# ROAM-Lab-ND/generalized_rbda

Hardware: AMD Instinct MI355X
Metric: forward-dynamics evals/sec (batched random states), MIT Humanoid cluster model (higher is better)
Workload: dtype f32; 1 GPU; mit_humanoid.urdf cluster-ABA, 262144 random states per GPU; batch_per_gpu=262144, batch_global=262144, nq=25, nv=24, n_bodies=37, n_clusters=17, parallelism=batch-sharded x1, plan replicated

## Files before the change

generalized_rbda_amd/csrc/capi.cpp:

```cpp
#include <hip/hip_runtime.h>

#include <array>
#include <cassert>
#include <cmath>
#include <cstdio>
#include <cstdlib>
#include <cstring>
#include <map>
#include <memory>
#include <mutex>
#include <string>
#include <vector>

#include "../../include/grbda_hip.h"
#include "../../include/grbda_hip_vjp.h"
#include "../../include/grbda_hip_step_vjp.h"
#include "../../include/grbda_hip_jvp.h"
#include "../../include/grbda_hip_wrench.h"
#include "../../include/grbda_hip_bodies.h"
#include "../../include/grbda_hip_jacobians.h"
#include "../../include/grbda_hip_jacobian_products.h"
#include "../../include/grbda_model_desc.h"
#include "devplan.h"

// ... 605 lines not shown
        if (int rc = ensure_scratch(p, device, stream, scratch_bytes(grid, static_cast<size_t>(d.n_glb_slots) + in_rows, sizeof(T)), &scratch)) return rc;
        hipError_t e = launch_aba_chain_lm<T>(d, q, qd, tau, ydd, B, static_cast<T *>(scratch), static_cast<int>(grid), lds_lm, hs, r.lm_waves);
        return e == hipSuccess ? GRBDA_OK : hip_err(e, "aba chain launch (latency mode)");
    }
    const int kid = sizeof(T) == 8 ? 1 : 0;
    const size_t waves_per_cu = static_cast<size_t>((sizeof(T) == 8 && !cp.gens.empty()) ? p->opt.waves_per_cu_f64_wide_regs : p->opt.waves_per_cu[kid]);
    const LaunchShape s = launch_shape(t.n_cu, n_tiles, waves_per_cu, static_cast<size_t>(cp.n_lds) * kWave * sizeof(T), h.nq, h.nv, sizeof(T),
                                       static_cast<size_t>(p->opt.lds_bytes_per_wave[kid]), true);
    {
        int n_free_bwd = 0, at_bwd = -1;
        for (size_t i = 0; i < cp.segs.size(); i++)
            if (cp.segs[i].op == SEG_FREE_BWD) { n_free_bwd++; at_bwd = static_cast<int>(i); }
        if (!cp.segs.empty() && cp.segs[0].op == SEG_FREE_FWD && n_free_bwd == 1 && cp.frees[cp.segs[0].first].lds_v >= 0) {
            if (s.stage_all_fits) d.fuse |= 1;
            d.stage_lds_v = cp.frees[cp.segs[0].first].lds_v;
            d.stage_v_index = cp.frees[cp.segs[0].first].v_index;
        }
        if (n_free_bwd == 1 && at_bwd + 1 < static_cast<int>(cp.segs.size()) && cp.segs[at_bwd + 1].op == SEG_FREE_ACC &&
            cp.segs[at_bwd + 1].first == cp.segs[at_bwd].first)
            d.fuse |= 2;
    }
    d.lds_bytes = static_cast<int>(s.lds_bytes);
    const bool inreg = !wrenches && chain_inputs_in_registers(sizeof(T), d.n_gens, d.n_diffs, d.sv_global, d.nq, d.nv);
    if (inreg) d.direct_in = chain_direct_inputs(sizeof(T), d.nq, d.nv, q, qd, tau);
    const size_t slab_rows = static_cast<size_t>(chain_slab_rows(inreg, d.nq, d.nv, d.n_glb_slots, d.out_lds).total);
    if (int rc = ensure_scratch(p, device, stream, scratch_bytes(s.grid, slab_rows, sizeof(T)), &scratch)) return rc;
    hipError_t e = wrenches ? launch_aba_chain_wrench<T>(d, *wrenches, q, qd, tau, ydd, B, static_cast<T *>(scratch), static_cast<int>(s.grid), s.lds_bytes, hs)
                            : launch_aba_chain<T>(d, q, qd, tau, ydd, B, static_cast<T *>(scratch), static_cast<int>(s.grid), s.lds_bytes, hs);
    return e == hipSuccess ? GRBDA_OK : hip_err(e, "aba chain launch");
}

template <class T>
int run_rnea_chain(const grbda_plan *p, const DeviceTables &t, const Route &r, const T *q, const T *qd, const T *ydd, T *tau, size_t B, int device,
                   void *stream, bool gravity = true, const WrenchList<T> *wrenches = nullptr)
{
    const HostPlan &h = p->host;
    const RneaChainProgram &rp = h.rchain[r.slot];
    const size_t n_tiles = (B + kWave - 1) / kWave;
    const size_t in_rows = static_cast<size_t>(h.nq + 2 * h.nv);
    const hipStream_t hs = static_cast<hipStream_t>(stream);
    RneaChainDev<T> d = rnea_chain_dev<T>(p, t, r.slot);
    if (!gravity)
        for (int i = 0; i < 6; i++) d.a_root[i] = T(0);
    void *scratch = nullptr;
    if (r.path == ROUTE_LM) {
        if (rp.diffs.empty()) d.diffs = nullptr;
        no_gens(d);
// ... 4045 lines not shown
```

generalized_rbda_amd/csrc/chain_kernels.hip:

```cpp
#include <hip/hip_runtime.h>

#include "devplan.h"

#ifndef GRBDA_CHAIN_UNIT
#define GRBDA_CHAIN_UNIT 0
#endif
#define GRBDA_KLDS (GRBDA_CHAIN_UNIT == 3)

namespace grbda_hip {

#include "devmath.h"

template <class T>
struct ChainTables {
    cptr<ChainSeg> segs;
    cptr<ChainLink> links;
    cptr<ChainPair> pairs;
    cptr<ChainFree> frees;
    cptr<ChainDiff> diffs;
    cptr<ChainGen> gens;
    cptr<ChainGenBody> gbodies;
    cptr<int32_t> cints;
    cptr<T> consts;
    int n_segs, nq, nv, ori_repr;
// ... 88 lines not shown
        if constexpr (sizeof(T) == 4) {
            if (out_row >= 0) reinterpret_cast<T *>(grbda_smem)[(out_row + j) * kWave + lane] = v;
            else put(j, v);
        } else {
            out_f[j * kWave + lane] = v;
        }
    }
    T *out_f;
    __device__ __forceinline__ void set_out(int row)
    {
        out_row = row;
        out_f = row >= 0 ? reinterpret_cast<T *>(grbda_smem) + row * kWave : out_u;
    }
    __device__ __forceinline__ void put(int j, T v) const
    {
        *reinterpret_cast<T *>(reinterpret_cast<char *>(out_u + (size_t)(unsigned)(j * kWave)) + (size_t)lane_b) = v;
    }
    __device__ __forceinline__ void wrench(int, T (&)[6]) const {}
};

template <class T>
struct ChainMemR : ChainMem<T> {
    typedef T Row __attribute__((ext_vector_type(kInRegCols)));
    Row rq, rqd, rx;
    __device__ __forceinline__ T q(int j) const { return rq[j]; }
    __device__ __forceinline__ T qd(int j) const { return rqd[j]; }
    __device__ __forceinline__ T x(int j) const { return rx[j]; }
};

template <class T>
struct ChainMemW : ChainMem<T> {
    int wbody[kMaxWrenches];
    unsigned wcanon;
    const T *wl;
    __device__ __forceinline__ void wrench(int body, T (&p)[6]) const
    {
        unsigned hits = 0;
#pragma unroll
        for (int i = 0; i < kMaxWrenches; i++) hits |= (wbody[i] == body ? 1u : 0u) << i;
        while (hits) {
            const int i = __builtin_ctz(hits);
            hits &= hits - 1;
            const T *w = wl + i * 6;
            const int shift = (int)((wcanon >> (2 * i)) & 3u) + 1;
#pragma unroll
            for (int j = 0; j < 3; j++) {
                const int k = (j + shift) % 3;
                p[j] -= w[k];
                p[3 + j] -= w[3 + k];
            }
// ... 343 lines not shown
#pragma unroll
    for (int j = 0; j < 6; j++) solve2(F0[j], F1[j], blk[j], blk[6 + j]);
    solve2(u[0], u[1], blk[12], blk[13]);
    M.glb_st(pr.glb_k, blk);
    if constexpr (OSIM) {
        const T ex[7] = {i00, i01, i11, s1, c1, s2, c2};
        M.glb_st(pr.glb_k + 14, ex);
    }
#pragma unroll
    for (int r = 0; r < 6; r++) {
        psi[r] += F0[r] * blk[12] + F1[r] * blk[13];
#pragma unroll
        for (int cc = r; cc < 6; cc++) IA[sidx(r, cc)] -= F0[r] * blk[cc] + F1[r] * blk[6 + cc];
    }
}
template <class T, bool OSIM, class MM>
__device__ __forceinline__ void pair_bwd(const ChainTables<T> &P, const MM &M, const ChainPair &pr, T (&IA)[21],
                                         T (&psi)[6])
{
    if (perm_if<T>(kPermPair, pr.perm[0]) == 0 && pr.perm[1] == 0) pair_bwd_k<T, OSIM, 0, 0>(P, M, pr, IA, psi);
    else pair_bwd_k<T, OSIM, -1, -1>(P, M, pr, IA, psi);
}

template <class T>
__device__ __forceinline__ void pair_acc(const ChainTables<T> &P, const ChainMem<T> &M, const ChainPair &pr)
{
    T blk[14], va[12];
    M.glb_ld(pr.glb_k, blk);
    M.lds_ld(pr.lds_pva, va);
    T y0 = blk[12], y1 = blk[13];
#pragma unroll
    for (int j = 0; j < 6; j++) {
        y0 -= blk[j] * va[6 + j];
        y1 -= blk[6 + j] * va[6 + j];
    }
    M.put_f(pr.v_index, y0);
    M.put_f(pr.v_index + 1, y1);
}


template <class T, class TB>
__device__ __forceinline__ void diff_constraint(const TB &P, const ChainMem<T> &M, int tofs_i, int lds_w, const T (&qs)[4], T yd0,
                                                T yd1, T (&X)[4], T (&g)[2], T (&qdl)[2])
{
    cptr<int32_t> ip = P.cints + tofs_i;
    const int n_args = ip[0], n_atoms = ip[1];
    cptr<T> dp = P.consts + ip[2];
    for (int i = 0; i < n_args; i++) {
// ... 542 lines not shown
#pragma unroll
                for (int j = 0; j < 8; j++) blk[j] = blkn[j];
            }
        }
    }
    if (sg.lds_acc_out != -1) {
        T acc[27];
        if (sg.acc_first) {
#pragma unroll
            for (int j = 0; j < 21; j++) acc[j] = IAc[j];
#pragma unroll
            for (int j = 0; j < 6; j++) acc[21 + j] = psic[j];
        } else {
            M.acc_ld(sg.lds_acc_out, acc);
#pragma unroll
            for (int j = 0; j < 21; j++) acc[j] += IAc[j];
#pragma unroll
            for (int j = 0; j < 6; j++) acc[21 + j] += psic[j];
        }
        M.acc_st(sg.lds_acc_out, acc);
    }
}

template <class T>
__device__ __forceinline__ void run_acc(const ChainTables<T> &P, const ChainMem<T> &M, const ChainSeg &sg)
{
    T vp[6], ap[6];
    if (sg.lds_pva >= 0) {
        T va[12];
        M.lds_ld(sg.lds_pva, va);
#pragma unroll
        for (int j = 0; j < 6; j++) {
            vp[j] = va[j];
            ap[j] = va[6 + j];
        }
    } else {
#pragma unroll
        for (int j = 0; j < 6; j++) {
            vp[j] = 0;
            ap[j] = P.a_root[j];
        }
    }
    ChainLink l = load_rec(P.links + sg.first);
    T kb[7];
    M.glb_ld(l.glb_k, kb);
    T yd = M.qd(l.v_index), yq = l.has_child ? M.q(l.q_index) : T(0);
    for (int i = 0; i < sg.count; i++) {
        const bool more = i + 1 < sg.count;
// ... 123 lines not shown
#pragma unroll
                    for (int j = 0; j < 6; j++) {
                        vp[j] = v[j];
                        ap[j] = a[j];
                    }
                }
            }
        }
    }
}

template <class T, class MM>
__device__ __forceinline__ void free_fwd(const ChainTables<T> &P, const MM &M, const ChainFree &f)
{
    if (f.lds_v < 0) return;
    T v[6];
#pragma unroll
    for (int j = 0; j < 6; j++) v[j] = M.qd(f.v_index + j);
    M.lds_st(f.lds_v, v);
}

template <class T, class MM>
__device__ __forceinline__ void free_acc_inputs(const ChainTables<T> &P, const MM &M, const ChainFree &f, T (&o)[4], T (&r)[3]);
template <class T>
__device__ __forceinline__ void free_acc_core(const ChainTables<T> &P, const ChainMem<T> &M, const ChainFree &f, const T (&y0)[6],
                                              const T (&o)[4], const T (&r)[3], const T (&vb)[6]);
template <class T, bool OSIM, class MM>
__device__ __forceinline__ void free_bwd(const ChainTables<T> &P, const MM &M, const ChainFree &f, bool fuse_acc = false)
{
    cptr<T> Ic = P.consts + f.bofs;
    cptr<T> Ib = P.consts + f.iofs;
    T v[6], psi[6], IA[21];
#pragma unroll
    for (int j = 0; j < 6; j++) v[j] = M.qd(f.v_index + j);
    T o_[4] = {0, 0, 0, 0}, r_[3] = {0, 0, 0};
    if constexpr (!OSIM) {
        if (fuse_acc) free_acc_inputs(P, M, f, o_, r_);
    }
    bias_force(Ic, v, psi);
    M.wrench(f.body, psi);
    if (f.lds_acc != -1) {
        T acc[27];
        M.acc_ld(f.lds_acc, acc);
#pragma unroll
        for (int j = 0; j < 21; j++) IA[j] = Ib[j] + acc[j];
#pragma unroll
        for (int j = 0; j < 6; j++) psi[j] += acc[21 + j];
        if (f.lds_acc2 != -1) {
// ... 34 lines not shown
    }
    M.glb_st(f.glb_y0, u);
    if constexpr (OSIM) {
        T ex[27];
#pragma unroll
        for (int i = 0; i < 6; i++) {
#pragma unroll
            for (int j = 0; j <= i; j++) ex[i * (i + 1) / 2 + j] = ch.L[i][j];
            ex[21 + i] = ch.inv[i];
        }
        M.glb_st(f.glb_y0 + 6, ex);
    }
}

template <class T, class MM>
__device__ __forceinline__ void free_acc_inputs(const ChainTables<T> &P, const MM &M, const ChainFree &f, T (&o)[4], T (&r)[3])
{
    const int nori = P.ori_repr == 0 ? 4 : 3;
#pragma unroll
    for (int j = 0; j < 4; j++) o[j] = j < nori ? M.q(f.q_index + 3 + j) : T(0);
#pragma unroll
    for (int j = 0; j < 3; j++) r[j] = M.q(f.q_index + j);
}
template <class T>
__device__ __forceinline__ void free_acc_core(const ChainTables<T> &P, const ChainMem<T> &M, const ChainFree &f, const T (&y0)[6],
                                              const T (&o)[4], const T (&r)[3], const T (&vb)[6])
{
    T E[9], g[6], ag[6];
    free_rotation(P.ori_repr, o, E);
#pragma unroll
    for (int j = 0; j < 6; j++) g[j] = P.a_root[j];
    xmotion(E, r, g, ag);
#pragma unroll
    for (int j = 0; j < 6; j++) M.put_f(f.v_index + j, y0[j] - ag[j]);
    if (f.lds_va >= 0) {
        T va[12];
#pragma unroll
        for (int j = 0; j < 6; j++) {
            va[j] = vb[j];
            va[6 + j] = y0[j];
        }
        M.lds_st(f.lds_va, va);
    }
}
template <class T, class MM>
__device__ __forceinline__ void free_acc(const ChainTables<T> &P, const MM &M, const ChainFree &f)
{
    T y0[6], o[4], r[3], vb[6];
// ... 119 lines not shown
template int gen1_waves_per_simd<float>(int);
template int gen1_waves_per_simd<double>(int);
template <class T>
hipError_t launch_aba_gen1(const ChainDev<T> &P, int n, int implicit, const T *q, const T *qd, const T *tau, T *ydd, size_t B, int grid,
                           size_t lds_bytes, hipStream_t stream)
{
    if (implicit) {
        if (n == 1) return launch_gen1<T, 1, true>(P, q, qd, tau, ydd, B, grid, lds_bytes, stream);
        if (n == 2) return launch_gen1<T, 2, true>(P, q, qd, tau, ydd, B, grid, lds_bytes, stream);
        if (n == 3) return launch_gen1<T, 3, true>(P, q, qd, tau, ydd, B, grid, lds_bytes, stream);
        return launch_gen1<T, 4, true>(P, q, qd, tau, ydd, B, grid, lds_bytes, stream);
    }
    if (n == 1) return launch_gen1<T, 1, false>(P, q, qd, tau, ydd, B, grid, lds_bytes, stream);
    if (n == 2) return launch_gen1<T, 2, false>(P, q, qd, tau, ydd, B, grid, lds_bytes, stream);
    if (n == 3) return launch_gen1<T, 3, false>(P, q, qd, tau, ydd, B, grid, lds_bytes, stream);
    return launch_gen1<T, 4, false>(P, q, qd, tau, ydd, B, grid, lds_bytes, stream);
}
template hipError_t launch_aba_gen1<float>(const ChainDev<float> &, int, int, const float *, const float *, const float *, float *, size_t, int,
                                           size_t, hipStream_t);
template hipError_t launch_aba_gen1<double>(const ChainDev<double> &, int, int, const double *, const double *, const double *, double *,
                                            size_t, int, size_t, hipStream_t);
#endif

template <class T, int WPS, int MODE, int DIRECT = 0>
__global__ __launch_bounds__(kWave, WPS) void aba_chain_kernel(ChainDev<T> DP, const T *__restrict__ q, const T *__restrict__ qd,
                                                             const T *__restrict__ tau, T *__restrict__ ydd, size_t B,
                                                             T *__restrict__ scratch)
{
    constexpr bool DIFF = MODE == 1 || MODE == 2, GEN = MODE == 2, INREG = MODE == kModeInReg;
    static_assert(INREG || DIRECT == 0, "direct row loads fill the register vectors of kModeInReg");
    ChainTables<T> P;
    P.segs = (cptr<ChainSeg>)DP.segs;
    P.links = (cptr<ChainLink>)DP.links;
    P.pairs = (cptr<ChainPair>)DP.pairs;
    P.frees = (cptr<ChainFree>)DP.frees;
    P.diffs = DIFF ? (cptr<ChainDiff>)DP.diffs : nullptr;
    P.gens = GEN ? (cptr<ChainGen>)DP.gens : nullptr;
    P.gbodies = GEN ? (cptr<ChainGenBody>)DP.gbodies : nullptr;
    P.cints = DIFF ? (cptr<int32_t>)DP.cints : nullptr;
    P.consts = (cptr<T>)DP.consts;
    P.n_segs = DP.n_segs;
    P.nq = DP.nq;
    P.nv = DP.nv;
    P.ori_repr = DP.ori_repr;
#pragma unroll
    for (int i = 0; i < 6; i++) P.a_root[i] = DP.a_root[i];
    const int lane = threadIdx.x;
    const ChainSlabRows rows = chain_slab_rows(INREG, P.nq, P.nv, DP.n_glb_slots, DP.out_lds);
    T *slab = scratch + (size_t)blockIdx.x * (size_t)rows.total * kWave;
    std::conditional_t<INREG, ChainMemR<T>, ChainMem<T>> M;
    M.lane = lane;
    M.lane_b = (unsigned)lane * (unsigned)sizeof(T);
    M.gmul = 1;
    M.amask = ~0;
    M.glb_u = slab + (size_t)rows.glb * kWave;
    M.in_q_u = slab;
    M.in_qd_u = slab + (size_t)P.nq * kWave;
    M.in_x_u = slab + (size_t)(P.nq + P.nv) * kWave;
    M.out_u = slab + (size_t)rows.out * kWave;
    M.set_out(DP.out_lds);
    M.bad = 0;

    const size_t n_tiles = (B + kWave - 1) / kWave;
    for (size_t tile = blockIdx.x; tile < n_tiles; tile += gridDim.x) {
        const size_t left = B - tile * kWave;
        const int rows_valid = left < (size_t)kWave ? (int)left : kWave;
        if constexpr (INREG)
            stage_inputs_reg<kInRegCols, (DIRECT & kDirectQ) != 0, (DIRECT & kDirectQd) != 0, (DIRECT & kDirectX) != 0>(
                q, qd, tau, tile, rows_valid, P.nq, P.nv, M.rq, M.rqd, M.rx, lane, DP.lds_bytes);
        else stage_inputs(q, qd, tau, tile, rows_valid, P.nq, P.nv, slab, lane, DP.lds_bytes);
        if (DP.fuse & 1) {
            T v[6];
            if constexpr ((DIRECT & kDirectQd) != 0) {
#pragma unroll
                for (int j = 0; j < 6; j++) v[j] = M.rqd[DP.stage_v_index + j];
            } else {
                const T *mine = reinterpret_cast<const T *>(grbda_smem) + (kWave * P.nq + lane * P.nv + DP.stage_v_index);
#pragma unroll
                for (int j = 0; j < 6; j++) v[j] = mine[j];
                wave_lds_fence();
            }
            M.lds_st(DP.stage_lds_v, v);
        }
        for (int s = 0; s < P.n_segs; s++) {
            const ChainSeg sg = load_rec(P.segs + s);
            switch (sg.op) {
                case SEG_RUN_FWD:
                    if (DP.sv_global) run_fwd<T, true>(P, M, sg);
                    else run_fwd_c(P, M, sg);
                    break;
                case SEG_RUN_BWD: {
                    if (DP.sv_global) run_bwd<T, false, true>(P, M, sg);
                    else if (sg.rot_kind == 1) run_bwd<T, false, false, 1>(P, M, sg);
                    else run_bwd<T, false, false>(P, M, sg);
                    break;
                }
// ... 8 lines not shown
                case SEG_DIFF_FWD:
                    if constexpr (DIFF) diff_fwd(P, M, load_rec(P.diffs + sg.first));
                    break;
                case SEG_DIFF_BWD:
                    if constexpr (DIFF) diff_bwd<T, false>(P, M, load_rec(P.diffs + sg.first));
                    break;
                case SEG_DIFF_ACC:
                    if constexpr (DIFF) diff_acc(P, M, load_rec(P.diffs + sg.first));
                    break;
                case SEG_GEN_FWD:
                    if constexpr (GEN) gen_segment<T, 0>(P, M, load_rec(P.gens + sg.first));
                    break;
                case SEG_GEN_BWD:
                    if constexpr (GEN) gen_segment<T, 1>(P, M, load_rec(P.gens + sg.first));
                    break;
                case SEG_GEN_ACC:
                    if constexpr (GEN) gen_segment<T, 2>(P, M, load_rec(P.gens + sg.first));
                    break;
                default:
                    if (!(DP.fuse & 2)) free_acc(P, M, load_rec(P.frees + sg.first));
                    break;
            }
        }
        if (M.out_row >= 0) write_outputs_lds<T>(M.out_row, ydd, tile, rows_valid, P.nv, lane);
        else write_outputs(slab + (size_t)rows.out * kWave, ydd, tile, rows_valid, P.nv, lane);
        M.flush_bad(DP.bad_count, rows_valid);
    }
}


template <class T, int NW, bool DIFF = false>
__global__ __launch_bounds__(NW * kWave) __attribute__((amdgpu_waves_per_eu(2, 2)))
void aba_chain_lm_kernel(ChainDev<T> DP, const T *__restrict__ q, const T *__restrict__ qd, const T *__restrict__ tau,
                         T *__restrict__ ydd, size_t B, T *__restrict__ scratch)
{
    ChainTables<T> P;
    P.segs = (cptr<ChainSeg>)DP.segs;
    P.links = (cptr<ChainLink>)DP.links;
    P.pairs = (cptr<ChainPair>)DP.pairs;
    P.frees = (cptr<ChainFree>)DP.frees;
    P.diffs = DIFF ? (cptr<ChainDiff>)DP.diffs : nullptr;
    P.gens = nullptr;
    P.gbodies = nullptr;
    P.cints = DIFF ? (cptr<int32_t>)DP.cints : nullptr;
    P.consts = (cptr<T>)DP.consts;
    P.n_segs = DP.n_segs;
    P.nq = DP.nq;
// ... 525 lines not shown
                                              double *, double *, size_t, double *, int, size_t, hipStream_t);
#endif

hipError_t launch_aba_chain_diff_f64(const ChainDev<double> &P, const double *q, const double *qd, const double *tau, double *ydd, size_t B,
                                     double *scratch, int grid, size_t lds_bytes, hipStream_t stream);
template <class T>
hipError_t launch_aba_chain_gen(const ChainDev<T> &P, const T *q, const T *qd, const T *tau, T *ydd, size_t B, T *scratch, int grid,
                                size_t lds_bytes, hipStream_t stream);
template <class T>
hipError_t launch_aba_chain(const ChainDev<T> &P, const T *q, const T *qd, const T *tau, T *ydd, size_t B, T *scratch, int grid,
                            size_t lds_bytes, hipStream_t stream)
{
    if (P.n_gens > 0) return launch_aba_chain_gen<T>(P, q, qd, tau, ydd, B, scratch, grid, lds_bytes, stream);
    if (P.n_diffs > 0) {
        if constexpr (sizeof(T) == 8) {
            return launch_aba_chain_diff_f64(P, q, qd, tau, ydd, B, scratch, grid, lds_bytes, stream);
        } else {
            hipLaunchKernelGGL((aba_chain_kernel<T, 2, 1>), dim3(grid), dim3(kWave), lds_bytes, stream, P, q, qd, tau, ydd, B, scratch);
            return hipGetLastError();
        }
    }
    if constexpr (sizeof(T) == 4) {
        if (chain_inputs_in_registers(sizeof(T), P.n_gens, P.n_diffs, P.sv_global, P.nq, P.nv)) {
            if (P.direct_in == (kDirectQ | kDirectQd | kDirectX))
                hipLaunchKernelGGL((aba_chain_kernel<T, 2, kModeInReg, kDirectQ | kDirectQd | kDirectX>), dim3(grid), dim3(kWave), lds_bytes, stream, P, q, qd,
                                   tau, ydd, B, scratch);
            else if (P.direct_in == (kDirectQd | kDirectX))
                hipLaunchKernelGGL((aba_chain_kernel<T, 2, kModeInReg, kDirectQd | kDirectX>), dim3(grid), dim3(kWave), lds_bytes, stream, P, q, qd, tau,
                                   ydd, B, scratch);
            else
                hipLaunchKernelGGL((aba_chain_kernel<T, 2, kModeInReg>), dim3(grid), dim3(kWave), lds_bytes, stream, P, q, qd, tau, ydd, B, scratch);
            return hipGetLastError();
        }
    }
    hipLaunchKernelGGL((aba_chain_kernel<T, 2, 0>), dim3(grid), dim3(kWave), lds_bytes, stream, P, q, qd, tau, ydd, B, scratch);
    return hipGetLastError();
}
#if GRBDA_CHAIN_UNIT == 0
template hipError_t launch_aba_chain<float>(const ChainDev<float> &, const float *, const float *, const float *, float *, size_t,
                                            float *, int, size_t, hipStream_t);
template hipError_t launch_aba_chain<double>(const ChainDev<double> &, const double *, const double *, const double *, double *,
                                             size_t, double *, int, size_t, hipStream_t);
#elif GRBDA_CHAIN_UNIT == 1
hipError_t launch_aba_chain_diff_f64(const ChainDev<double> &P, const double *q, const double *qd, const double *tau, double *ydd, size_t B,
                                     double *scratch, int grid, size_t lds_bytes, hipStream_t stream)
{
    hipLaunchKernelGGL((aba_chain_kernel<double, 2, 1>), dim3(grid), dim3(kWave), lds_bytes, stream, P, q, qd, tau, ydd, B, scratch);
    return hipGetLastError();
}
#elif GRBDA_CHAIN_UNIT == 2
template <class T>
hipError_t launch_aba_chain_gen(const ChainDev<T> &P, const T *q, const T *qd, const T *tau, T *ydd, size_t B, T *scratch, int grid,
                                size_t lds_bytes, hipStream_t stream)
{
// ... 874 lines not shown
                                                    const float *, float *, size_t, float *, int, size_t, hipStream_t);
template hipError_t launch_rnea_chain_wrench<double>(const RneaChainDev<double> &, const WrenchList<double> &, int, const double *, const double *,
                                                     const double *, double *, size_t, double *, int, size_t, hipStream_t);
#endif


static hipError_t set_max_dynamic_lds(const void *const *kernels, int n)
{
    for (int i = 0; i < n; i++) {
        const hipError_t e = hipFuncSetAttribute(kernels[i], hipFuncAttributeMaxDynamicSharedMemorySize, 160 * 1024);
        if (e != hipSuccess) return e;
    }
    return hipSuccess;
}
hipError_t set_max_dynamic_lds_chain_unit1();
hipError_t set_max_dynamic_lds_chain_unit2();
hipError_t set_max_dynamic_lds_chain_unit3();
#if GRBDA_CHAIN_UNIT == 0
hipError_t set_max_dynamic_lds_chain()
{
    const void *const kernels[] = {
        reinterpret_cast<const void *>(&aba_chain_kernel<float, 2, 0>), reinterpret_cast<const void *>(&aba_chain_kernel<float, 2, 1>),
        reinterpret_cast<const void *>(&aba_chain_kernel<float, 2, kModeInReg>),
        reinterpret_cast<const void *>(&aba_chain_kernel<float, 2, kModeInReg, kDirectQd | kDirectX>),
        reinterpret_cast<const void *>(&aba_chain_kernel<float, 2, kModeInReg, kDirectQ | kDirectQd | kDirectX>),
        reinterpret_cast<const void *>(&aba_chain_kernel<double, 2, 0>),
        reinterpret_cast<const void *>(&rnea_chain_kernel<float, 0, false>), reinterpret_cast<const void *>(&rnea_chain_kernel<float, 1, false>),
        reinterpret_cast<const void *>(&rnea_chain_kernel<double, 0, false>), reinterpret_cast<const void *>(&rnea_chain_kernel<double, 1, false>),
        reinterpret_cast<const void *>(&rnea_chain_kernel<float, 0, true>), reinterpret_cast<const void *>(&rnea_chain_kernel<float, 1, true>),
        reinterpret_cast<const void *>(&rnea_chain_kernel<double, 0, true>), reinterpret_cast<const void *>(&rnea_chain_kernel<double, 1, true>),
        reinterpret_cast<const void *>(&osim_chain_kernel<float>), reinterpret_cast<const void *>(&osim_chain_kernel<double>)};
    const hipError_t e = set_max_dynamic_lds(kernels, static_cast<int>(sizeof(kernels) / sizeof(kernels[0])));
    if (e != hipSuccess) return e;
    const hipError_t e1 = set_max_dynamic_lds_chain_unit1();
    if (e1 != hipSuccess) return e1;
    const hipError_t e2 = set_max_dynamic_lds_chain_unit2();
    return e2 != hipSuccess ? e2 : set_max_dynamic_lds_chain_unit3();
}
#elif GRBDA_CHAIN_UNIT == 1
hipError_t set_max_dynamic_lds_chain_unit1()
{
    const void *const kernels[] = {reinterpret_cast<const void *>(&aba_chain_kernel<double, 2, 1>),
                                   reinterpret_cast<const void *>(&aba_chain_lm_kernel<double, 2>)};
    return set_max_dynamic_lds(kernels, 2);
}
#elif GRBDA_CHAIN_UNIT == 3
hipError_t set_max_dynamic_lds_chain_unit3()
{
// ... 31 lines not shown
```

generalized_rbda_amd/csrc/devmath.h:

```cpp
#pragma once

template <class U>
using cptr = const U __attribute__((address_space(4))) *;

template <class U>
__device__ __forceinline__ U load_rec(cptr<U> p)
{
    static_assert(sizeof(U) % 4 == 0, "plan records are arrays of int32");
    U out;
    cptr<int32_t> src = (cptr<int32_t>)p;
    int32_t *dst = reinterpret_cast<int32_t *>(&out);
#pragma unroll
    for (int i = 0; i < (int)(sizeof(U) / 4); i++) dst[i] = src[i];
    return out;
}

extern __shared__ __attribute__((aligned(16))) unsigned char grbda_smem[];

__host__ __device__ constexpr int sidx(int i, int j)
{
    return i <= j ? (i * 6 - i * (i - 1) / 2 + (j - i)) : (j * 6 - j * (j - 1) / 2 + (i - j));
}

template <class T>
// ... 356 lines not shown
        stage_transpose(nq, 0u, slab, lane);
        stage_transpose(nv, bq, slab + (size_t)nq * kWave, lane);
        stage_transpose(nv, bq + bv, slab + (size_t)(nq + nv) * kWave, lane);
        wave_lds_fence();
    } else {
        stage_issue(q, tile, rows_valid, nq, 0u, lane);
        asm volatile("s_waitcnt vmcnt(0)" ::: "memory");
        wave_lds_fence();
        stage_transpose(nq, 0u, slab, lane);
        wave_lds_fence();
        stage_issue(qd, tile, rows_valid, nv, 0u, lane);
        asm volatile("s_waitcnt vmcnt(0)" ::: "memory");
        wave_lds_fence();
        stage_transpose(nv, 0u, slab + (size_t)nq * kWave, lane);
        wave_lds_fence();
        stage_issue(x, tile, rows_valid, nv, 0u, lane);
        asm volatile("s_waitcnt vmcnt(0)" ::: "memory");
        wave_lds_fence();
        stage_transpose(nv, 0u, slab + (size_t)(nq + nv) * kWave, lane);
        wave_lds_fence();
    }
}

template <class T, int N, class ROW>
__device__ __forceinline__ void stage_row_regs(int ncols, unsigned lds_byte_off, ROW &r, int lane)
{
    const T *stage = reinterpret_cast<const T *>(grbda_smem + lds_byte_off);
    constexpr int V = 16 / (int)sizeof(T);
    static_assert(N % V == 0, "whole 16-byte reads");
    if ((ncols % V) == 0 && (lds_byte_off % 16u) == 0) {
        struct alignas(16) Vec { T v[V]; };
        const Vec *rows = reinterpret_cast<const Vec *>(stage + lane * ncols);
#pragma unroll
        for (int c = 0; c < N; c += V) {
            if (c < ncols) {
                const Vec x = rows[c / V];
#pragma unroll
                for (int k = 0; k < V; k++) r[c + k] = x.v[k];
            }
        }
        return;
    }
#pragma unroll
    for (int c = 0; c < N; c++)
        if (c < ncols) r[c] = stage[lane * ncols + c];
}
template <class T, int N, class ROW>
__device__ __forceinline__ void load_row_regs(const T *__restrict__ src, size_t tile, int rows_valid, int ncols, ROW &r, int lane)
{
    constexpr int V = 16 / (int)sizeof(T);
    static_assert(N % V == 0, "whole 16-byte loads");
    struct alignas(16) Vec { T v[V]; };
    const int row = lane < rows_valid ? lane : rows_valid - 1;
    const Vec *mine = reinterpret_cast<const Vec *>(src + (tile * (size_t)kWave + (size_t)row) * (size_t)ncols);
    const int last = ncols / V - 1;
#pragma unroll
    for (int c = 0; c < N; c += V) {
        const Vec x = mine[c / V < last ? c / V : last];
#pragma unroll
        for (int k = 0; k < V; k++) r[c + k] = x.v[k];
    }
}
template <int K>
__device__ __forceinline__ void wait_all_but_youngest()
{
    static_assert(K >= 0 && K < 64, "six bits of vmcnt");
    asm volatile("s_waitcnt vmcnt(%0)" ::"n"(K) : "memory");
}
template <int N, bool DQ, bool DQD, bool DX, class T, class ROW>
__device__ __forceinline__ void stage_inputs_reg(const T *__restrict__ q, const T *__restrict__ qd, const T *__restrict__ x, size_t tile,
                                                 int rows_valid, int nq, int nv, ROW &rq, ROW &rqd, ROW &rx, int lane, int lds_bytes)
{
    constexpr int V = 16 / (int)sizeof(T), kDirectLoads = ((DQ ? 1 : 0) + (DQD ? 1 : 0) + (DX ? 1 : 0)) * (N / V);
    const unsigned bq = (unsigned)(kWave * nq) * (unsigned)sizeof(T), bv = (unsigned)(kWave * nv) * (unsigned)sizeof(T);
    if ((int)(bq + 2 * bv) <= lds_bytes) {
        if constexpr (!DQ) stage_issue(q, tile, rows_valid, nq, 0u, lane);
        if constexpr (!DQD) stage_issue(qd, tile, rows_valid, nv, bq, lane);
        if constexpr (!DX) stage_issue(x, tile, rows_valid, nv, bq + bv, lane);
        if constexpr (kDirectLoads > 0) asm volatile("" ::: "memory");
        if constexpr (DQ) load_row_regs<T, N>(q, tile, rows_valid, nq, rq, lane);
        if constexpr (DQD) load_row_regs<T, N>(qd, tile, rows_valid, nv, rqd, lane);
        if constexpr (DQD && DX) asm volatile("" ::: "memory");
        if constexpr (DX) load_row_regs<T, N>(x, tile, rows_valid, nv, rx, lane);
        if constexpr (DQ && DQD && DX) return;
        wait_all_but_youngest<kDirectLoads>();
        wave_lds_fence();
        if constexpr (!DQ) stage_row_regs<T, N>(nq, 0u, rq, lane);
        if constexpr (!DQD) stage_row_regs<T, N>(nv, bq, rqd, lane);
        if constexpr (!DX) stage_row_regs<T, N>(nv, bq + bv, rx, lane);
        wave_lds_fence();
    } else {
        if constexpr (DQ) load_row_regs<T, N>(q, tile, rows_valid, nq, rq, lane);
        if constexpr (DQD) load_row_regs<T, N>(qd, tile, rows_valid, nv, rqd, lane);
        if constexpr (DX) load_row_regs<T, N>(x, tile, rows_valid, nv, rx, lane);
        if constexpr (!DQ) {
            stage_issue(q, tile, rows_valid, nq, 0u, lane);
            asm volatile("s_waitcnt vmcnt(0)" ::: "memory");
            wave_lds_fence();
            stage_row_regs<T, N>(nq, 0u, rq, lane);
            wave_lds_fence();
        }
        if constexpr (!DQD) {
            stage_issue(qd, tile, rows_valid, nv, 0u, lane);
            asm volatile("s_waitcnt vmcnt(0)" ::: "memory");
            wave_lds_fence();
            stage_row_regs<T, N>(nv, 0u, rqd, lane);
            wave_lds_fence();
        }
        if constexpr (!DX) {
            stage_issue(x, tile, rows_valid, nv, 0u, lane);
            asm volatile("s_waitcnt vmcnt(0)" ::: "memory");
            wave_lds_fence();
            stage_row_regs<T, N>(nv, 0u, rx, lane);
            wave_lds_fence();
        }
    }
}

template <class T>
__device__ __forceinline__ void write_outputs(const T *rows, T *__restrict__ out, size_t tile, int rows_valid, int nv,
                                              int lane)
{
    asm volatile("s_waitcnt vmcnt(0) lgkmcnt(0)" ::: "memory");
    T *stage = reinterpret_cast<T *>(grbda_smem);
    constexpr int V = 16 / (int)sizeof(T);
    if ((nv % V) == 0) {
        struct alignas(16) Vec { T v[V]; };
        Vec *mine = reinterpret_cast<Vec *>(stage + lane * nv);
        for (int c = 0; c < nv; c += V) {
            Vec x;
#pragma unroll
            for (int k = 0; k < V; k++) x.v[k] = rows[(size_t)(c + k) * kWave + lane];
            mine[c / V] = x;
        }
    } else {
        for (int c = 0; c < nv; c++) stage[lane * nv + c] = rows[(size_t)c * kWave + lane];
    }
    wave_lds_fence();
    T *dst = out + tile * (size_t)kWave * (size_t)nv;
// ... 193 lines not shown
```

generalized_rbda_amd/csrc/devplan.h:

```cpp
#pragma once
#include <cstdlib>
#include <hip/hip_runtime.h>

#include "plan.h"
#include "walk.h"

namespace grbda_hip {

inline size_t lds_workgroups_per_cu(size_t lds_bytes)
{
    if (lds_bytes == 0) return 32;
    constexpr size_t granule = 1280;
    return (160u * 1024u) / ((lds_bytes + granule - 1) / granule * granule);
}


template <class T>
struct DevPlan {
    const Step *steps;
    int n_steps;
    const ClusterRec *clusters;
    const BodyRec *bodies;
    const T *consts;
    const int32_t *cints;
// ... 40 lines not shown
template <class T>
hipError_t launch_twists(const DevPlan<T> &P, int n_clusters, int n_span, const T *q, const T *qd_span, const T *qdd_span, T *V, size_t B,
                         int grid, hipStream_t stream);
hipError_t set_max_dynamic_lds();

template <class T>
struct ChainDev {
    const ChainSeg *segs;
    const ChainLink *links;
    const ChainPair *pairs;
    const ChainFree *frees;
    const ChainDiff *diffs;
    int n_diffs;
    const ChainGen *gens;
    const ChainGenBody *gbodies;
    int n_gens;
    const int32_t *cints;
    const T *consts;
    int n_segs;
    int nq, nv;
    int n_glb_slots;
    int lds_bytes;
    int ori_repr;
    int direct_in;
    int sv_global;
    int out_lds;
    int fuse, stage_lds_v, stage_v_index;
    unsigned long long *bad_count;
    T a_root[6];
};
constexpr int kInRegCols = 32;
constexpr int kModeInReg = 3;
inline bool chain_inputs_in_registers(size_t elem, int n_gens, int n_diffs, int sv_global, int nq, int nv)
{
    return elem == 4 && n_gens == 0 && n_diffs == 0 && !sv_global && nq <= kInRegCols && nv <= kInRegCols;
}
constexpr int kDirectQ = 1, kDirectQd = 2, kDirectX = 4;
inline int chain_direct_inputs(size_t elem, int nq, int nv, const void *q, const void *qd, const void *x)
{
    const auto direct = [elem](int ncols, const void *base) {
        return (static_cast<size_t>(ncols) * elem) % 16 == 0 && reinterpret_cast<uintptr_t>(base) % 16 == 0;
    };
    if (!direct(nv, qd) || !direct(nv, x)) return 0;
    return kDirectQd | kDirectX | (direct(nq, q) ? kDirectQ : 0);
}
struct ChainSlabRows {
    int glb;
    int out;
    int total;
};
__host__ __device__ inline ChainSlabRows chain_slab_rows(bool in_registers, int nq, int nv, int n_glb_slots, int out_lds)
{
    if (!in_registers) return {nq + 2 * nv, nq + nv, nq + 2 * nv + n_glb_slots};
    return {0, out_lds < 0 ? n_glb_slots : 0, n_glb_slots + (out_lds < 0 ? nv : 0)};
}
template <class T>
hipError_t launch_aba_chain(const ChainDev<T> &P, const T *q, const T *qd, const T *tau, T *ydd, size_t B, T *scratch, int grid,
                            size_t lds_bytes, hipStream_t stream);
template <class T>
hipError_t launch_aba_chain_lm(const ChainDev<T> &P, const T *q, const T *qd, const T *tau, T *ydd, size_t B, T *scratch, int grid,
                               size_t lds_bytes, hipStream_t stream, int n_waves);
hipError_t set_max_dynamic_lds_chain();
template <class T>
hipError_t launch_aba_gen1(const ChainDev<T> &P, int n, int implicit, const T *q, const T *qd, const T *tau, T *ydd, size_t B, int grid,
                           size_t lds_bytes, hipStream_t stream);
template <class T>
int gen1_waves_per_simd(int n);
// ... 275 lines not shown
```

Baseline: 2.322 billion evals/s.

## Load chain inputs directly into registers and write outputs from registers

Result: faster. 2.481 billion evals/s, median of 6 (+6.9%).

```diff
diff --git a/generalized_rbda_amd/csrc/capi.cpp b/generalized_rbda_amd/csrc/capi.cpp
--- a/generalized_rbda_amd/csrc/capi.cpp
+++ b/generalized_rbda_amd/csrc/capi.cpp
@@ -651,7 +651,6 @@
     }
     d.lds_bytes = static_cast<int>(s.lds_bytes);
     const bool inreg = !wrenches && chain_inputs_in_registers(sizeof(T), d.n_gens, d.n_diffs, d.sv_global, d.nq, d.nv);
-    if (inreg) d.direct_in = chain_direct_inputs(sizeof(T), d.nq, d.nv, q, qd, tau);
     const size_t slab_rows = static_cast<size_t>(chain_slab_rows(inreg, d.nq, d.nv, d.n_glb_slots, d.out_lds).total);
     if (int rc = ensure_scratch(p, device, stream, scratch_bytes(s.grid, slab_rows, sizeof(T)), &scratch)) return rc;
     hipError_t e = wrenches ? launch_aba_chain_wrench<T>(d, *wrenches, q, qd, tau, ydd, B, static_cast<T *>(scratch), static_cast<int>(s.grid), s.lds_bytes, hs)
diff --git a/generalized_rbda_amd/csrc/chain_kernels.hip b/generalized_rbda_amd/csrc/chain_kernels.hip
--- a/generalized_rbda_amd/csrc/chain_kernels.hip
+++ b/generalized_rbda_amd/csrc/chain_kernels.hip
@@ -134,10 +134,14 @@
 template <class T>
 struct ChainMemR : ChainMem<T> {
     typedef T Row __attribute__((ext_vector_type(kInRegCols)));
-    Row rq, rqd, rx;
+    Row rq, rqd;
+    mutable Row rx;
     __device__ __forceinline__ T q(int j) const { return rq[j]; }
     __device__ __forceinline__ T qd(int j) const { return rqd[j]; }
     __device__ __forceinline__ T x(int j) const { return rx[j]; }
+    __device__ __forceinline__ void put_f(int j, T v) const { rx[j] = v; }
+    void put(int, T) const = delete;
+    T got(int) const = delete;
 };
 
 template <class T>
@@ -527,8 +531,8 @@
     else pair_bwd_k<T, OSIM, -1, -1>(P, M, pr, IA, psi);
 }
 
-template <class T>
-__device__ __forceinline__ void pair_acc(const ChainTables<T> &P, const ChainMem<T> &M, const ChainPair &pr)
+template <class T, class MM>
+__device__ __forceinline__ void pair_acc(const ChainTables<T> &P, const MM &M, const ChainPair &pr)
 {
     T blk[14], va[12];
     M.glb_ld(pr.glb_k, blk);
@@ -1117,8 +1121,8 @@
     }
 }
 
-template <class T>
-__device__ __forceinline__ void run_acc(const ChainTables<T> &P, const ChainMem<T> &M, const ChainSeg &sg)
+template <class T, class MM>
+__device__ __forceinline__ void run_acc(const ChainTables<T> &P, const MM &M, const ChainSeg &sg)
 {
     T vp[6], ap[6];
     if (sg.lds_pva >= 0) {
@@ -1288,8 +1292,8 @@
 
 template <class T, class MM>
 __device__ __forceinline__ void free_acc_inputs(const ChainTables<T> &P, const MM &M, const ChainFree &f, T (&o)[4], T (&r)[3]);
-template <class T>
-__device__ __forceinline__ void free_acc_core(const ChainTables<T> &P, const ChainMem<T> &M, const ChainFree &f, const T (&y0)[6],
+template <class T, class MM>
+__device__ __forceinline__ void free_acc_core(const ChainTables<T> &P, const MM &M, const ChainFree &f, const T (&y0)[6],
                                               const T (&o)[4], const T (&r)[3], const T (&vb)[6]);
 template <class T, bool OSIM, class MM>
 __device__ __forceinline__ void free_bwd(const ChainTables<T> &P, const MM &M, const ChainFree &f, bool fuse_acc = false)
@@ -1370,8 +1374,8 @@
 #pragma unroll
     for (int j = 0; j < 3; j++) r[j] = M.q(f.q_index + j);
 }
-template <class T>
-__device__ __forceinline__ void free_acc_core(const ChainTables<T> &P, const ChainMem<T> &M, const ChainFree &f, const T (&y0)[6],
+template <class T, class MM>
+__device__ __forceinline__ void free_acc_core(const ChainTables<T> &P, const MM &M, const ChainFree &f, const T (&y0)[6],
                                               const T (&o)[4], const T (&r)[3], const T (&vb)[6])
 {
     T E[9], g[6], ag[6];
@@ -1537,13 +1541,12 @@
                                             size_t, int, size_t, hipStream_t);
 #endif
 
-template <class T, int WPS, int MODE, int DIRECT = 0>
+template <class T, int WPS, int MODE>
 __global__ __launch_bounds__(kWave, WPS) void aba_chain_kernel(ChainDev<T> DP, const T *__restrict__ q, const T *__restrict__ qd,
                                                              const T *__restrict__ tau, T *__restrict__ ydd, size_t B,
                                                              T *__restrict__ scratch)
 {
     constexpr bool DIFF = MODE == 1 || MODE == 2, GEN = MODE == 2, INREG = MODE == kModeInReg;
-    static_assert(INREG || DIRECT == 0, "direct row loads fill the register vectors of kModeInReg");
     ChainTables<T> P;
     P.segs = (cptr<ChainSeg>)DP.segs;
     P.links = (cptr<ChainLink>)DP.links;
@@ -1580,13 +1583,11 @@
     for (size_t tile = blockIdx.x; tile < n_tiles; tile += gridDim.x) {
         const size_t left = B - tile * kWave;
         const int rows_valid = left < (size_t)kWave ? (int)left : kWave;
-        if constexpr (INREG)
-            stage_inputs_reg<kInRegCols, (DIRECT & kDirectQ) != 0, (DIRECT & kDirectQd) != 0, (DIRECT & kDirectX) != 0>(
-                q, qd, tau, tile, rows_valid, P.nq, P.nv, M.rq, M.rqd, M.rx, lane, DP.lds_bytes);
+        if constexpr (INREG) load_inputs_reg<kInRegCols>(q, qd, tau, tile, rows_valid, P.nq, P.nv, M.rq, M.rqd, M.rx, lane);
         else stage_inputs(q, qd, tau, tile, rows_valid, P.nq, P.nv, slab, lane, DP.lds_bytes);
         if (DP.fuse & 1) {
             T v[6];
-            if constexpr ((DIRECT & kDirectQd) != 0) {
+            if constexpr (INREG) {
 #pragma unroll
                 for (int j = 0; j < 6; j++) v[j] = M.rqd[DP.stage_v_index + j];
             } else {
@@ -1641,7 +1642,8 @@
                     break;
             }
         }
-        if (M.out_row >= 0) write_outputs_lds<T>(M.out_row, ydd, tile, rows_valid, P.nv, lane);
+        if constexpr (INREG) store_row_regs<T, kInRegCols>(ydd, tile, rows_valid, P.nv, M.rx, lane);
+        else if (M.out_row >= 0) write_outputs_lds<T>(M.out_row, ydd, tile, rows_valid, P.nv, lane);
         else write_outputs(slab + (size_t)rows.out * kWave, ydd, tile, rows_valid, P.nv, lane);
         M.flush_bad(DP.bad_count, rows_valid);
     }
@@ -2213,14 +2215,7 @@
     }
     if constexpr (sizeof(T) == 4) {
         if (chain_inputs_in_registers(sizeof(T), P.n_gens, P.n_diffs, P.sv_global, P.nq, P.nv)) {
-            if (P.direct_in == (kDirectQ | kDirectQd | kDirectX))
-                hipLaunchKernelGGL((aba_chain_kernel<T, 2, kModeInReg, kDirectQ | kDirectQd | kDirectX>), dim3(grid), dim3(kWave), lds_bytes, stream, P, q, qd,
-                                   tau, ydd, B, scratch);
-            else if (P.direct_in == (kDirectQd | kDirectX))
-                hipLaunchKernelGGL((aba_chain_kernel<T, 2, kModeInReg, kDirectQd | kDirectX>), dim3(grid), dim3(kWave), lds_bytes, stream, P, q, qd, tau,
-                                   ydd, B, scratch);
-            else
-                hipLaunchKernelGGL((aba_chain_kernel<T, 2, kModeInReg>), dim3(grid), dim3(kWave), lds_bytes, stream, P, q, qd, tau, ydd, B, scratch);
+            hipLaunchKernelGGL((aba_chain_kernel<T, 2, kModeInReg>), dim3(grid), dim3(kWave), lds_bytes, stream, P, q, qd, tau, ydd, B, scratch);
             return hipGetLastError();
         }
     }
@@ -3141,8 +3136,6 @@
     const void *const kernels[] = {
         reinterpret_cast<const void *>(&aba_chain_kernel<float, 2, 0>), reinterpret_cast<const void *>(&aba_chain_kernel<float, 2, 1>),
         reinterpret_cast<const void *>(&aba_chain_kernel<float, 2, kModeInReg>),
-        reinterpret_cast<const void *>(&aba_chain_kernel<float, 2, kModeInReg, kDirectQd | kDirectX>),
-        reinterpret_cast<const void *>(&aba_chain_kernel<float, 2, kModeInReg, kDirectQ | kDirectQd | kDirectX>),
         reinterpret_cast<const void *>(&aba_chain_kernel<double, 2, 0>),
         reinterpret_cast<const void *>(&rnea_chain_kernel<float, 0, false>), reinterpret_cast<const void *>(&rnea_chain_kernel<float, 1, false>),
         reinterpret_cast<const void *>(&rnea_chain_kernel<double, 0, false>), reinterpret_cast<const void *>(&rnea_chain_kernel<double, 1, false>),
diff --git a/generalized_rbda_amd/csrc/devmath.h b/generalized_rbda_amd/csrc/devmath.h
--- a/generalized_rbda_amd/csrc/devmath.h
+++ b/generalized_rbda_amd/csrc/devmath.h
@@ -402,99 +402,80 @@
     }
 }
 
-template <class T, int N, class ROW>
-__device__ __forceinline__ void stage_row_regs(int ncols, unsigned lds_byte_off, ROW &r, int lane)
-{
-    const T *stage = reinterpret_cast<const T *>(grbda_smem + lds_byte_off);
-    constexpr int V = 16 / (int)sizeof(T);
-    static_assert(N % V == 0, "whole 16-byte reads");
-    if ((ncols % V) == 0 && (lds_byte_off % 16u) == 0) {
-        struct alignas(16) Vec { T v[V]; };
-        const Vec *rows = reinterpret_cast<const Vec *>(stage + lane * ncols);
-#pragma unroll
-        for (int c = 0; c < N; c += V) {
-            if (c < ncols) {
-                const Vec x = rows[c / V];
-#pragma unroll
-                for (int k = 0; k < V; k++) r[c + k] = x.v[k];
-            }
-        }
-        return;
-    }
-#pragma unroll
-    for (int c = 0; c < N; c++)
-        if (c < ncols) r[c] = stage[lane * ncols + c];
+template <class T, int V>
+struct alignas(sizeof(T)) RowUnit {
+    T v[V];
+};
+__device__ __forceinline__ int tile_local(int ncols)
+{
+    asm volatile("" : "+s"(ncols));
+    return ncols;
 }
 template <class T, int N, class ROW>
 __device__ __forceinline__ void load_row_regs(const T *__restrict__ src, size_t tile, int rows_valid, int ncols, ROW &r, int lane)
 {
     constexpr int V = 16 / (int)sizeof(T);
-    static_assert(N % V == 0, "whole 16-byte loads");
-    struct alignas(16) Vec { T v[V]; };
+    static_assert(N % V == 0, "whole 16-byte units");
     const int row = lane < rows_valid ? lane : rows_valid - 1;
-    const Vec *mine = reinterpret_cast<const Vec *>(src + (tile * (size_t)kWave + (size_t)row) * (size_t)ncols);
-    const int last = ncols / V - 1;
+    const T *mine = src + (tile * (size_t)kWave + (size_t)row) * (size_t)ncols;
+    const int n = tile_local(ncols), wide = n - n % V;
 #pragma unroll
     for (int c = 0; c < N; c += V) {
-        const Vec x = mine[c / V < last ? c / V : last];
-#pragma unroll
-        for (int k = 0; k < V; k++) r[c + k] = x.v[k];
-    }
-}
-template <int K>
-__device__ __forceinline__ void wait_all_but_youngest()
-{
-    static_assert(K >= 0 && K < 64, "six bits of vmcnt");
-    asm volatile("s_waitcnt vmcnt(%0)" ::"n"(K) : "memory");
-}
-template <int N, bool DQ, bool DQD, bool DX, class T, class ROW>
-__device__ __forceinline__ void stage_inputs_reg(const T *__restrict__ q, const T *__restrict__ qd, const T *__restrict__ x, size_t tile,
-                                                 int rows_valid, int nq, int nv, ROW &rq, ROW &rqd, ROW &rx, int lane, int lds_bytes)
-{
-    constexpr int V = 16 / (int)sizeof(T), kDirectLoads = ((DQ ? 1 : 0) + (DQD ? 1 : 0) + (DX ? 1 : 0)) * (N / V);
-    const unsigned bq = (unsigned)(kWave * nq) * (unsigned)sizeof(T), bv = (unsigned)(kWave * nv) * (unsigned)sizeof(T);
-    if ((int)(bq + 2 * bv) <= lds_bytes) {
-        if constexpr (!DQ) stage_issue(q, tile, rows_valid, nq, 0u, lane);
-        if constexpr (!DQD) stage_issue(qd, tile, rows_valid, nv, bq, lane);
-        if constexpr (!DX) stage_issue(x, tile, rows_valid, nv, bq + bv, lane);
-        if constexpr (kDirectLoads > 0) asm volatile("" ::: "memory");
-        if constexpr (DQ) load_row_regs<T, N>(q, tile, rows_valid, nq, rq, lane);
-        if constexpr (DQD) load_row_regs<T, N>(qd, tile, rows_valid, nv, rqd, lane);
-        if constexpr (DQD && DX) asm volatile("" ::: "memory");
-        if constexpr (DX) load_row_regs<T, N>(x, tile, rows_valid, nv, rx, lane);
-        if constexpr (DQ && DQD && DX) return;
-        wait_all_but_youngest<kDirectLoads>();
-        wave_lds_fence();
-        if constexpr (!DQ) stage_row_regs<T, N>(nq, 0u, rq, lane);
-        if constexpr (!DQD) stage_row_regs<T, N>(nv, bq, rqd, lane);
-        if constexpr (!DX) stage_row_regs<T, N>(nv, bq + bv, rx, lane);
-        wave_lds_fence();
-    } else {
-        if constexpr (DQ) load_row_regs<T, N>(q, tile, rows_valid, nq, rq, lane);
-        if constexpr (DQD) load_row_regs<T, N>(qd, tile, rows_valid, nv, rqd, lane);
-        if constexpr (DX) load_row_regs<T, N>(x, tile, rows_valid, nv, rx, lane);
-        if constexpr (!DQ) {
-            stage_issue(q, tile, rows_valid, nq, 0u, lane);
-            asm volatile("s_waitcnt vmcnt(0)" ::: "memory");
-            wave_lds_fence();
-            stage_row_regs<T, N>(nq, 0u, rq, lane);
-            wave_lds_fence();
-        }
-        if constexpr (!DQD) {
-            stage_issue(qd, tile, rows_valid, nv, 0u, lane);
-            asm volatile("s_waitcnt vmcnt(0)" ::: "memory");
-            wave_lds_fence();
-            stage_row_regs<T, N>(nv, 0u, rqd, lane);
-            wave_lds_fence();
-        }
-        if constexpr (!DX) {
-            stage_issue(x, tile, rows_valid, nv, 0u, lane);
-            asm volatile("s_waitcnt vmcnt(0)" ::: "memory");
-            wave_lds_fence();
-            stage_row_regs<T, N>(nv, 0u, rx, lane);
-            wave_lds_fence();
-        }
-    }
+        if (c < wide) {
+            const RowUnit<T, V> x = *reinterpret_cast<const RowUnit<T, V> *>(mine + c);
+#pragma unroll
+            for (int k = 0; k < V; k++) r[c + k] = x.v[k];
+        }
+    }
+    if (wide == n) return;
+#pragma unroll
+    for (int c = 0; c < N; c += V) {
+        if (c == wide) {
+#pragma unroll
+            for (int k = 0; k < V - 1; k++)
+                if (c + k < n) r[c + k] = mine[c + k];
+        }
+    }
+}
+constexpr int kWaitVmcnt0 = (0x7 << 4) | (0xf << 8);
+static_assert(kWaitVmcnt0 == 0x0f70, "vmcnt(0) expcnt(7) lgkmcnt(15)");
+template <class T, int N, class ROW>
+__device__ __forceinline__ void store_row_regs(T *__restrict__ dst, size_t tile, int rows_valid, int ncols, const ROW &r, int lane)
+{
+    constexpr int V = 16 / (int)sizeof(T);
+    static_assert(N % V == 0, "whole 16-byte units");
+    __builtin_amdgcn_s_waitcnt(kWaitVmcnt0);
+    if (lane >= rows_valid) return;
+    T *mine = dst + (tile * (size_t)kWave + (size_t)lane) * (size_t)ncols;
+    const int n = tile_local(ncols), wide = n - n % V;
+#pragma unroll
+    for (int c = 0; c < N; c += V) {
+        if (c < wide) {
+            RowUnit<T, V> x;
+#pragma unroll
+            for (int k = 0; k < V; k++) x.v[k] = r[c + k];
+            *reinterpret_cast<RowUnit<T, V> *>(mine + c) = x;
+        }
+    }
+    if (wide == n) return;
+#pragma unroll
+    for (int c = 0; c < N; c += V) {
+        if (c == wide) {
+#pragma unroll
+            for (int k = 0; k < V - 1; k++)
+                if (c + k < n) mine[c + k] = r[c + k];
+        }
+    }
+}
+template <int N, class T, class ROW>
+__device__ __forceinline__ void load_inputs_reg(const T *__restrict__ q, const T *__restrict__ qd, const T *__restrict__ x, size_t tile,
+                                                int rows_valid, int nq, int nv, ROW &rq, ROW &rqd, ROW &rx, int lane)
+{
+    load_row_regs<T, N>(q, tile, rows_valid, nq, rq, lane);
+    asm volatile("" ::: "memory");
+    load_row_regs<T, N>(qd, tile, rows_valid, nv, rqd, lane);
+    asm volatile("" ::: "memory");
+    load_row_regs<T, N>(x, tile, rows_valid, nv, rx, lane);
 }
 
 template <class T>
diff --git a/generalized_rbda_amd/csrc/devplan.h b/generalized_rbda_amd/csrc/devplan.h
--- a/generalized_rbda_amd/csrc/devplan.h
+++ b/generalized_rbda_amd/csrc/devplan.h
@@ -86,7 +86,6 @@
     int n_glb_slots;
     int lds_bytes;
     int ori_repr;
-    int direct_in;
     int sv_global;
     int out_lds;
     int fuse, stage_lds_v, stage_v_index;
@@ -98,15 +97,6 @@
 inline bool chain_inputs_in_registers(size_t elem, int n_gens, int n_diffs, int sv_global, int nq, int nv)
 {
     return elem == 4 && n_gens == 0 && n_diffs == 0 && !sv_global && nq <= kInRegCols && nv <= kInRegCols;
-}
-constexpr int kDirectQ = 1, kDirectQd = 2, kDirectX = 4;
-inline int chain_direct_inputs(size_t elem, int nq, int nv, const void *q, const void *qd, const void *x)
-{
-    const auto direct = [elem](int ncols, const void *base) {
-        return (static_cast<size_t>(ncols) * elem) % 16 == 0 && reinterpret_cast<uintptr_t>(base) % 16 == 0;
-    };
-    if (!direct(nv, qd) || !direct(nv, x)) return 0;
-    return kDirectQd | kDirectX | (direct(nq, q) ? kDirectQ : 0);
 }
 struct ChainSlabRows {
     int glb;
```
